# eridgd/WCT-TF

Hardware: AMD Instinct MI355X
Metric: stylized frames/sec @512x512, 5-level relu5->1 pipeline, alpha=0.8 (higher is better)
Workload: dtype f16

## Files before the change

wct_tf_amd/csrc/conv_wino.hip:

```cpp
#include "common.h"
#include "conv_tile.h"

namespace {
template <int TH, int BN, int WM, int WN>
struct WinoShape {
  static constexpr int PR = TH / 2;
  static constexpr int MT = (PR / 2) / WM;
  static constexpr int NT = (BN / 32) / WN;
  static constexpr int G = 256 / PR;
  static constexpr int SL = (72 + G - 1) / G;
  static constexpr int PATCH_BYTES = PR * 4 * PITCH * 64;
  static_assert(PR % 2 == 0 && (PR / 2) % WM == 0 && 256 % PR == 0 && WM * WN == 4, "tile shape");
  static constexpr int DUMP_OFF = 2 * PATCH_BYTES;
  static constexpr int BIAS_OFF = DUMP_OFF + 8192;
  static size_t patch_lds_bytes() { return 2 * (size_t)PATCH_BYTES; }
  static size_t lds_bytes(int cout) { return BIAS_OFF + 4 * (size_t)cout; }
};

__device__ __forceinline__ half8 pk_sub(half8 a, half8 b) {
  u32x4 ua = __builtin_bit_cast(u32x4, a), ub = __builtin_bit_cast(u32x4, b), r;
#pragma unroll
  for (int i = 0; i < 4; ++i) {
    unsigned o;
    asm("v_pk_add_f16 %0, %1, %2 neg_lo:[0,1] neg_hi:[0,1]" : "=v"(o) : "v"(ua[i]), "v"(ub[i]));
    r[i] = o;
  }
  return __builtin_bit_cast(half8, r);
}

__device__ __forceinline__ half8 wino_T(const u32x4 (&raw)[4], int f) {
  const half8 d0 = __builtin_bit_cast(half8, raw[0]), d1 = __builtin_bit_cast(half8, raw[1]);
  const half8 d2 = __builtin_bit_cast(half8, raw[2]), d3 = __builtin_bit_cast(half8, raw[3]);
  return f == 0 ? pk_sub(d0, d2) : f == 1 ? d1 + d2 : f == 2 ? pk_sub(d2, d1) : pk_sub(d1, d3);
}

__device__ __forceinline__ void wino_row_offsets(ConvArgs p, int Win, int y0, int lpr, unsigned (&row_off)[4]) {
#pragma unroll
  for (int i = 0; i < 4; ++i) {
    int iy = reflect_idx(y0 + 2 * lpr - 1 + i, p.H);
    if (p.upsample) iy >>= 1;
    row_off[i] = (unsigned)(iy * Win) * p.Cin * 2;
  }
}
__device__ __forceinline__ int wino_slot_px(int slot) { return slot < 72 ? slot >> 2 : 0; }
__device__ __forceinline__ unsigned wino_col_offset(ConvArgs p, int x0, int slot) {
  int ix = reflect_idx(x0 - 1 + wino_slot_px(slot), p.W);
  if (p.upsample) ix >>= 1;
  return (unsigned)(ix * p.Cin + (slot & 3) * 8) * 2;
}
__device__ __forceinline__ unsigned wino_slot_dst(int lpr, int slot) {
  const int px = wino_slot_px(slot), piece = slot & 3;
  return ((lpr * 4 * PITCH + px) * 4 + (piece ^ ((px >> 2) & 3))) * 16;
}

template <int MT>
__device__ __forceinline__ void wino_rd_base(int (&rd_base)[3][2], int wm, int frag_px, int frag_pr, int kgrp) {
#pragma unroll
  for (int kx = 0; kx < 3; ++kx)
#pragma unroll
    for (int ks = 0; ks < 2; ++ks) {
      const int px = frag_px + kx;
      rd_base[kx][ks] = (((wm * MT * 2 + frag_pr) * 4) * PITCH + px) * 64 + (((ks * 2 + kgrp) ^ ((px >> 2) & 3)) * 16);
    }
}
__device__ __forceinline__ half8 wino_pixel_frag(const unsigned char* patch, const int (&rd_base)[3][2], int f, int kx, int ks, int mt) {
  return *reinterpret_cast<const half8*>(patch + rd_base[kx][ks] + (mt * 8 + f) * PITCH * 64);
}
template <int MT>
__device__ __forceinline__ void wino_read_b(half8 (&dst)[2][MT], const unsigned char* patch, const int (&rd_base)[3][2], int f, int kx) {
#pragma unroll
  for (int ks = 0; ks < 2; ++ks)
#pragma unroll
    for (int mt = 0; mt < MT; ++mt) dst[ks][mt] = wino_pixel_frag(patch, rd_base, f, kx, ks, mt);
}
template <int NT>
__device__ __forceinline__ void wino_wfrag(unsigned (&wfrag)[NT], int ctile0, int wn, int c16, int lane) {
#pragma unroll
  for (int nt = 0; nt < NT; ++nt) wfrag[nt] = ((ctile0 + wn * NT + nt) * 12 * c16 * 512 + lane * 8) * 2;
}
__device__ __forceinline__ int wino_w_soff(int c16, int tap12, int chunk, unsigned wt) { return (tap12 * c16 + chunk * 2) * 1024 + wt; }
__device__ __forceinline__ half8 wino_weight_frag(__amdgpu_buffer_rsrc_t w_rsrc, unsigned wfrag, int ks, int soff) {
  return __builtin_bit_cast(half8, __builtin_amdgcn_raw_buffer_load_b128(w_rsrc, wfrag + ks * 1024, soff, 0));
}
template <int NT>
__device__ __forceinline__ void wino_load_w(half8 (&dst)[NT][2], __amdgpu_buffer_rsrc_t w_rsrc, const unsigned (&wfrag)[NT], int soff) {
#pragma unroll
  for (int nt = 0; nt < NT; ++nt)
#pragma unroll
    for (int ks = 0; ks < 2; ++ks) dst[nt][ks] = wino_weight_frag(w_rsrc, wfrag[nt], ks, soff);
}

template <int MT, int NT>
__device__ __forceinline__ void wino_init_acc(f32x16 (&acc)[4][NT][MT], const f32x4 (&bv)[NT][4]) {
#pragma unroll
  for (int nt = 0; nt < NT; ++nt)
#pragma unroll
    for (int f = 0; f < 4; ++f)
#pragma unroll
      for (int mt = 0; mt < MT; ++mt)
#pragma unroll
        for (int r = 0; r < 16; ++r) acc[f][nt][mt][r] = f == 1 ? bv[nt][r >> 2][r & 3] : 0.f;
}

template <int MT, int NT>
__device__ __forceinline__ void wino_epilogue(ConvArgs p, f32x16 (&acc)[4][NT][MT], int b, int y0, int x0, int n0, int wm, int wn,
                                              int frag_px, int frag_pr, int kgrp, int relu) {
  constexpr int OOB = (int)0x80000000u;
  const int Ho = p.pool ? (p.H + 1) / 2 : p.H, Wo = p.pool ? (p.W + 1) / 2 : p.W;
  const unsigned img_elems = (unsigned)Ho * Wo * p.Cout;
  const __amdgpu_buffer_rsrc_t r16 = __builtin_amdgcn_make_buffer_rsrc((void*)(p.y16 + (size_t)b * img_elems), 0, img_elems * 2, 0x00020000);
  const float lo1 = relu ? 0.f : -__builtin_inff();
  const h2 lo2 = {(half_t)lo1, (half_t)lo1};
  const h2 zero2 = {(half_t)0.f, (half_t)0.f};
  const int ox = x0 + frag_px;
  const int chan = n0 + wn * NT * 32;
#pragma unroll
  for (int mt = 0; mt < MT; ++mt) {
    const int oy = y0 + ((wm * MT + mt) * 2 + frag_pr) * 2;
    const bool in0 = (oy < p.H) & (ox < p.W), in1 = (oy + 1 < p.H) & (ox < p.W);
    int off[2];
    if (p.pool) {
      off[0] = in0 && (frag_px & 1) == 0 ? (((oy >> 1) * Wo + (ox >> 1)) * p.Cout + chan + 8 * kgrp) * 2 : OOB;
      off[1] = OOB;
    } else {
      off[0] = in0 ? ((oy * p.W + ox) * p.Cout + chan + 8 * kgrp) * 2 : OOB;
      off[1] = in1 ? (((oy + 1) * p.W + ox) * p.Cout + chan + 8 * kgrp) * 2 : OOB;
    }
#pragma unroll
    for (int nt = 0; nt < NT; ++nt) {
      unsigned pk[2][4][2];
#pragma unroll
      for (int rq = 0; rq < 4; ++rq) {
        f32x4 e, o;
#pragma unroll
        for (int j = 0; j < 4; ++j) {
          const int r = rq * 4 + j;
          const float m0 = acc[0][nt][mt][r], m1 = acc[1][nt][mt][r], m2 = acc[2][nt][mt][r], m3 = acc[3][nt][mt][r];
          e[j] = (m0 + m1) + m2;
          o[j] = (m1 - m2) - m3;
        }
        h2 e0 = {(half_t)e[0], (half_t)e[1]}, e1 = {(half_t)e[2], (half_t)e[3]};
        h2 o0 = {(half_t)o[0], (half_t)o[1]}, o1 = {(half_t)o[2], (half_t)o[3]};
        e0 = __builtin_elementwise_max(e0, lo2); e1 = __builtin_elementwise_max(e1, lo2);
        o0 = __builtin_elementwise_max(o0, lo2); o1 = __builtin_elementwise_max(o1, lo2);
        if (p.pool) {
          h2 q[2] = {__builtin_elementwise_max(in0 ? e0 : zero2, in1 ? o0 : zero2), __builtin_elementwise_max(in0 ? e1 : zero2, in1 ? o1 : zero2)};
#pragma unroll
          for (int d = 0; d < 2; ++d) {
            const unsigned tq = __builtin_bit_cast(unsigned, q[d]);
            const h2 nb = __builtin_bit_cast(h2, __builtin_amdgcn_update_dpp(0, (int)tq, 0xB1, 0xF, 0xF, true));
            q[d] = __builtin_elementwise_max(q[d], nb);
          }
          e0 = q[0]; e1 = q[1];
        }
        pk[0][rq][0] = __builtin_bit_cast(unsigned, e0); pk[0][rq][1] = __builtin_bit_cast(unsigned, e1);
        pk[1][rq][0] = __builtin_bit_cast(unsigned, o0); pk[1][rq][1] = __builtin_bit_cast(unsigned, o1);
      }
#pragma unroll
      for (int par = 0; par < 2; ++par) {
#pragma unroll
        for (int m = 0; m < 2; ++m) {
          auto sx = __builtin_amdgcn_permlane32_swap(pk[par][2 * m][0], pk[par][2 * m + 1][0], false, false);
          auto sy = __builtin_amdgcn_permlane32_swap(pk[par][2 * m][1], pk[par][2 * m + 1][1], false, false);
          u32x4 ov = {sx[0], sy[0], sx[1], sy[1]};
          __builtin_amdgcn_raw_buffer_store_b128(ov, r16, off[par] + (nt * 32 + 16 * m) * 2, 0, 0);
        }
      }
    }
  }
}

template <int TH, int BN, int WM, int WN>
__global__ __launch_bounds__(256, 2)
void conv3x3_wino_kernel(ConvArgs p, int tiles_x, int n_tiles) {
  using S = WinoShape<TH, BN, WM, WN>;
  constexpr int MT = S::MT, NT = S::NT, G = S::G, SL = S::SL;
  constexpr int PF_TAP = 5;
  static_assert(TH == 8, "two blocks per CU: the 8-row shapes only");

  extern __shared__ __attribute__((aligned(16))) unsigned char smem[];
  const int tid = threadIdx.x, lane = tid & 63, wave = tid >> 6;
  const int wm = wave / WN, wn = wave % WN;
  int bid = blockIdx.x;
  const int ntile = bid % n_tiles;
  bid /= n_tiles;
  const int tx = bid % tiles_x, ty = bid / tiles_x;
  const int b = blockIdx.y;
  const int y0 = ty * TH, x0 = tx * TW, n0 = ntile * BN;

  const int Hin = p.upsample ? p.H / 2 : p.H;
  const int Win = p.upsample ? p.W / 2 : p.W;
  const half_t* xb = p.x + (size_t)b * Hin * Win * p.Cin;
  const __amdgpu_buffer_rsrc_t w_rsrc = __builtin_amdgcn_make_buffer_rsrc((void*)p.w_wino, 0, 0x7FFFFFFF, 0x00020000);
  const __amdgpu_buffer_rsrc_t x_rsrc = __builtin_amdgcn_make_buffer_rsrc((void*)xb, 0, 0x7FFFFFFF, 0x00020000);

  const int lpr = tid / G, ls = tid % G;
  unsigned row_off[4], col_off[SL], dst_off[SL];
  bool slot_ok[SL];
  wino_row_offsets(p, Win, y0, lpr, row_off);
#pragma unroll
  for (int j = 0; j < SL; ++j) {
    const int slot = ls + j * G;
    slot_ok[j] = slot < 72;
    col_off[j] = wino_col_offset(p, x0, slot);
    dst_off[j] = wino_slot_dst(lpr, slot);
  }
  u32x4 raw[SL][4];
  auto load_rows = [&](int chunk) {
#pragma unroll
    for (int j = 0; j < SL; ++j)
#pragma unroll
      for (int i = 0; i < 4; ++i)
        raw[j][i] = __builtin_amdgcn_raw_buffer_load_b128(x_rsrc, row_off[i] + col_off[j], chunk * BK * 2, 0);
  };
  auto park_rows = [&](int buf) {
#pragma unroll
    for (int j = 0; j < SL; ++j) {
      const half8 t0 = wino_T(raw[j], 0), t1 = wino_T(raw[j], 1), t2 = wino_T(raw[j], 2), t3 = wino_T(raw[j], 3);
      if (slot_ok[j]) {
        unsigned char* d = smem + buf * S::PATCH_BYTES + dst_off[j];
        *reinterpret_cast<half8*>(d) = t0;
        *reinterpret_cast<half8*>(d + PITCH * 64) = t1;
        *reinterpret_cast<half8*>(d + 2 * PITCH * 64) = t2;
        *reinterpret_cast<half8*>(d + 3 * PITCH * 64) = t3;
      }
    }
  };

  const int frag_px = lane & 15, frag_pr = (lane & 31) >> 4, kgrp = lane >> 5;
  int rd_base[3][2];
  wino_rd_base<MT>(rd_base, wm, frag_px, frag_pr, kgrp);
  const int c16 = p.Cin >> 4;
  unsigned wfrag[NT];
  wino_wfrag<NT>(wfrag, n0 >> 5, wn, c16, lane);
  f32x16 acc[4][NT][MT];
  f32x4 bv[NT][4];
#pragma unroll
  for (int nt = 0; nt < NT; ++nt)
#pragma unroll
    for (int rq = 0; rq < 4; ++rq) bv[nt][rq] = *reinterpret_cast<const f32x4*>(p.bias + n0 + (wn * NT + nt) * 32 + 8 * rq + 4 * kgrp);
  wino_init_acc<MT, NT>(acc, bv);

  const int n_chunks = p.Cin / BK;
  half8 wf[3][NT][2];
  half8 bf[2][2][MT];
  auto load_w = [&](half8 (&dst)[NT][2], int tap12, int chunk) { wino_load_w<NT>(dst, w_rsrc, wfrag, wino_w_soff(c16, tap12, chunk, 0)); };
  auto read_b = [&](half8 (&dst)[2][MT], int f, int kx, int buf) { wino_read_b<MT>(dst, smem + buf * S::PATCH_BYTES, rd_base, f, kx); };

  load_rows(0);
  load_w(wf[0], 0, 0);
  load_w(wf[1], 1, 0);
  park_rows(0);
  asm volatile("s_waitcnt lgkmcnt(0)\n\ts_barrier" ::: "memory");
  read_b(bf[0], 0, 0, 0);

#pragma unroll 1
  for (int pair = 0; pair < n_chunks; pair += 2) {
#pragma unroll
    for (int t = 0; t < 24; ++t) {
      const int tt = t % 12, chunk_i = pair + t / 12, buf = t / 12;
      const int f = tt / 3;
      const bool more = chunk_i + 1 < n_chunks;
      {
        const int t2 = (tt + 2) % 12;
        const int c2 = tt + 2 >= 12 ? (more ? chunk_i + 1 : chunk_i) : chunk_i;
        load_w(wf[(t + 2) % 3], t2, c2);
      }
      if (tt == PF_TAP && more) load_rows(chunk_i + 1);
      if (tt != 11) read_b(bf[(t + 1) & 1], (tt + 1) / 3, (tt + 1) % 3, buf);
      else if (more) read_b(bf[(t + 1) & 1], 0, 0, buf ^ 1);
      __builtin_amdgcn_sched_barrier(0);
#pragma unroll
      for (int ks = 0; ks < 2; ++ks)
#pragma unroll
        for (int mt = 0; mt < MT; ++mt)
#pragma unroll
          for (int nt = 0; nt < NT; ++nt)
            acc[f][nt][mt] = __builtin_amdgcn_mfma_f32_32x32x16_f16(wf[t % 3][nt][ks], bf[t & 1][ks][mt], acc[f][nt][mt], 0, 0, 0);
      __builtin_amdgcn_sched_barrier(0);
      if (tt == 10 && more) {
        park_rows(buf ^ 1);
        asm volatile("s_waitcnt lgkmcnt(0)\n\ts_barrier" ::: "memory");
      }
    }
  }

  wino_epilogue<MT, NT>(p, acc, b, y0, x0, n0, wm, wn, frag_px, frag_pr, kgrp, p.relu);
}

template <int TH, int BN, int WM, int WN>
__global__ __launch_bounds__(256, 1)
void conv3x3_wino_walk_kernel(ConvArgs p, int tiles_x, int n_tiles, int tiles_y, int n_total) {
  using S = WinoShape<TH, BN, WM, WN>;
  constexpr int MT = S::MT, NT = S::NT, G = S::G, SL = S::SL;

  extern __shared__ __attribute__((aligned(16))) unsigned char smem[];
  const int tid = threadIdx.x, lane = tid & 63, wave = tid >> 6;
  const int wave_s = __builtin_amdgcn_readfirstlane(wave);
  auto fresh_tid = [&]() {
    int v;
    asm volatile("v_mbcnt_lo_u32_b32 %0, -1, 0\n\tv_mbcnt_hi_u32_b32 %0, -1, %0" : "=v"(v));
    return wave_s * 64 + v;
  };
  const int wm = wave / WN, wn = wave % WN;
  struct Tile { int b, y0, x0, n0; };
  auto tile_at = [&](int t) {
    Tile r;
    r.n0 = (t % n_tiles) * BN;
    t /= n_tiles;
    r.x0 = (t % tiles_x) * TW;
    t /= tiles_x;
    r.y0 = (t % tiles_y) * TH;
    r.b = t / tiles_y;
    return r;
  };
  Tile cur = tile_at(blockIdx.x);

  const int Hin = p.upsample ? p.H / 2 : p.H;
  const int Win = p.upsample ? p.W / 2 : p.W;
  const __amdgpu_buffer_rsrc_t w_rsrc = __builtin_amdgcn_make_buffer_rsrc((void*)p.w_wino, 0, 0x7FFFFFFF, 0x00020000);
  auto image_rsrc = [&](int b) { return __builtin_amdgcn_make_buffer_rsrc((void*)(p.x + (size_t)b * Hin * Win * p.Cin), 0, 0x7FFFFFFF, 0x00020000); };
  __amdgpu_buffer_rsrc_t x_rsrc = image_rsrc(cur.b);

  const int lpr = tid / G, ls = tid % G;
  unsigned row_off[4], col_off[SL], dst_off[SL];
  bool slot_ok[SL];
  auto stage_from = [&](int y0, int x0) {
    const int tid_s = fresh_tid(), lpr = tid_s / G, ls = tid_s % G;
    wino_row_offsets(p, Win, y0, lpr, row_off);
#pragma unroll
    for (int j = 0; j < SL; ++j) col_off[j] = wino_col_offset(p, x0, ls + j * G);
  };
  stage_from(cur.y0, cur.x0);
#pragma unroll
  for (int j = 0; j < SL; ++j) {
    const int slot = ls + j * G;
    slot_ok[j] = slot < 72;
    dst_off[j] = wino_slot_dst(lpr, slot);
    if (!slot_ok[j]) dst_off[j] = S::DUMP_OFF + tid * 16;
  }
  u32x4 raw[SL][4];
  auto load_rows = [&](int chunk) {
#pragma unroll
    for (int j = 0; j < SL; ++j)
#pragma unroll
      for (int i = 0; i < 4; ++i)
        raw[j][i] = __builtin_amdgcn_raw_buffer_load_b128(x_rsrc, row_off[i] + col_off[j], chunk * BK * 2, 0);
  };

  const int frag_px = lane & 15, frag_pr = (lane & 31) >> 4, kgrp = lane >> 5;
  int rd_base[3][2];
  wino_rd_base<MT>(rd_base, wm, frag_px, frag_pr, kgrp);
  const int c16 = p.Cin >> 4;
  unsigned wfrag[NT];
  wino_wfrag<NT>(wfrag, 0, wn, c16, lane);
  auto wtile_off = [&](int n0) { return (unsigned)((n0 >> 5) * 12 * c16 * 1024); };

  f32x16 acc[4][NT][MT];
  const int n_chunks = p.Cin / BK;
  half8 bf[3][2][MT];

  int tile = blockIdx.x;
  Tile nxt = cur;
  unsigned wt_cur = wtile_off(cur.n0), wt_nxt = wt_cur;
  bool has_next = false;
  constexpr int WR = 4, WA = WR - 1;
  static_assert(24 % WR == 0, "ring");
  half8 wq[WR][NT][2];
  half8 tq[4];
  {
    load_rows(0);
#pragma unroll
    for (int i = 0; i < WA; ++i) wino_load_w<NT>(wq[i], w_rsrc, wfrag, wino_w_soff(c16, i, 0, wt_cur));
#pragma unroll
    for (int j = 0; j < SL; ++j) {
      unsigned char* d = smem + dst_off[j];
      *reinterpret_cast<half8*>(d) = wino_T(raw[j], 0);
      *reinterpret_cast<half8*>(d + PITCH * 64) = wino_T(raw[j], 1);
      *reinterpret_cast<half8*>(d + 2 * PITCH * 64) = wino_T(raw[j], 2);
      *reinterpret_cast<half8*>(d + 3 * PITCH * 64) = wino_T(raw[j], 3);
    }
    for (int c = tid * 4; c < p.Cout; c += 1024) *reinterpret_cast<f32x4*>(smem + S::BIAS_OFF + c * 4) = *reinterpret_cast<const f32x4*>(p.bias + c);
    asm volatile("s_waitcnt lgkmcnt(0)\n\ts_barrier" ::: "memory");
  }
#pragma unroll 1
  for (;;) {
  {
    constexpr int NM = 2 * MT * NT;
    constexpr int NR = 2 * NT + 2 * MT;
    constexpr int LT0 = 1, PT0 = 6;
    static_assert(LT0 + SL <= PT0 && PT0 + SL <= 10, "staging schedule");
    has_next = tile + (int)gridDim.x < n_total;
    wino_read_b<MT>(bf[0], smem, rd_base, 0, 0);
    wino_read_b<MT>(bf[1], smem, rd_base, 0, 1);
    {
      const int tid_b = fresh_tid(), wn = (tid_b >> 6) % WN, kgrp = (tid_b & 63) >> 5;
      f32x4 bv[NT][4];
#pragma unroll
      for (int nt = 0; nt < NT; ++nt)
#pragma unroll
        for (int rq = 0; rq < 4; ++rq) bv[nt][rq] = *reinterpret_cast<const f32x4*>(smem + S::BIAS_OFF + (cur.n0 + (wn * NT + nt) * 32 + 8 * rq + 4 * kgrp) * 4);
      wino_init_acc<MT, NT>(acc, bv);
    }
#pragma unroll 1
    for (int pair = 0;;) {
      int stage_c = pair + 2;
      unsigned stage_wt = wt_cur;
#pragma unroll
      for (int t = 0; t < 24; ++t) {
        const int tt = t % 12, chunk_i = pair + t / 12, buf = t / 12;
        const int f = tt / 3;
        if (t == 12 && pair + 2 >= n_chunks) {
          stage_c = pair + 1;
          if (has_next) {
            nxt = tile_at(tile + (int)gridDim.x);
            stage_c = 0;
            stage_wt = wt_nxt = wtile_off(nxt.n0);
            stage_from(nxt.y0, nxt.x0);
            x_rsrc = image_rsrc(nxt.b);
          }
        }
        const int chunk_n = t < 12 ? pair + 1 : stage_c;
        const unsigned wt_n = t < 12 ? wt_cur : stage_wt;
        const int t3 = (tt + WA) % 12, c3 = tt + WA >= 12 ? chunk_n : chunk_i;
        const int t1 = (tt + 2) % 12, buf1 = tt >= 10 ? buf ^ 1 : buf;
        const int soff3 = wino_w_soff(c16, t3, c3, tt + WA >= 12 ? wt_n : wt_cur);
#pragma unroll
        for (int j = 0; j < NM; ++j) {
          const int ks = j / (MT * NT), mt = (j / NT) % MT, nt = j % NT;
          acc[f][nt][mt] = __builtin_amdgcn_mfma_f32_32x32x16_f16(wq[t % WR][nt][ks], bf[t % 3][ks][mt], acc[f][nt][mt], 0, 0, 0);
#pragma unroll
          for (int k = j * NR / NM; k < (j + 1) * NR / NM; ++k) {
            if (k < 2 * NT) {
              wq[(t + WA) % WR][k / 2][k % 2] = wino_weight_frag(w_rsrc, wfrag[k / 2], k % 2, soff3);
            } else {
              const int kk = k - 2 * NT, ks1 = kk / MT, mt1 = kk % MT;
              bf[(t + 2) % 3][ks1][mt1] = wino_pixel_frag(smem + buf1 * S::PATCH_BYTES, rd_base, t1 / 3, t1 % 3, ks1, mt1);
            }
          }
          if (tt >= LT0 && tt < LT0 + SL) {
            const int sl = tt - LT0;
            if (j < 4) raw[sl][j] = __builtin_amdgcn_raw_buffer_load_b128(x_rsrc, row_off[j] + col_off[sl], chunk_n * BK * 2, 0);
          }
          if (tt >= PT0 && tt < PT0 + SL) {
            const int sl = tt - PT0;
#pragma unroll
            for (int it = j * 8 / NM; it < (j + 1) * 8 / NM; ++it) {
              const int fq = it >> 1;
              if ((it & 1) == 0) tq[fq] = wino_T(raw[sl], fq);
              else *reinterpret_cast<half8*>(smem + (buf ^ 1) * S::PATCH_BYTES * (slot_ok[sl] ? 1 : 0) + dst_off[sl] + fq * PITCH * 64) = tq[fq];
            }
          }
          __builtin_amdgcn_sched_barrier(0);
        }
        if (tt == 9) asm volatile("s_waitcnt lgkmcnt(0)\n\ts_barrier" ::: "memory");
      }
      if ((pair += 2) >= n_chunks) break;
    }
  }
  const int tid_e = fresh_tid();
  const int lane_e = tid_e & 63, wn = (tid_e >> 6) % WN, wm = (tid_e >> 6) / WN;
  int relu = p.relu;
  asm volatile("" : "+s"(relu));
  wino_epilogue<MT, NT>(p, acc, cur.b, cur.y0, cur.x0, cur.n0, wm, wn, lane_e & 15, (lane_e & 31) >> 4, lane_e >> 5, relu);
  if (!has_next) break;
  tile += gridDim.x;
  cur = nxt;
  wt_cur = wt_nxt;
  }
}

template <int TH, int BN, int WM, int WN>
int launch_wino_cfg(const ConvArgs& a, hipStream_t s) {
  const int tiles_x = cdiv(a.W, TW), tiles_y = cdiv(a.H, TH), n_tiles = a.Cout / BN;
  const size_t lds = WinoShape<TH, BN, WM, WN>::patch_lds_bytes();
  HIP_TRY(hipFuncSetAttribute(reinterpret_cast<const void*>(&conv3x3_wino_kernel<TH, BN, WM, WN>),
                              hipFuncAttributeMaxDynamicSharedMemorySize, (int)lds));
  hipLaunchKernelGGL((conv3x3_wino_kernel<TH, BN, WM, WN>), dim3(tiles_x * tiles_y * n_tiles, a.B), dim3(256), lds, s, a, tiles_x, n_tiles);
  HIP_TRY(hipGetLastError());
  return WCT_OK;
}

template <int TH, int BN, int WM, int WN>
int launch_wino_walk(const ConvArgs& a, hipStream_t s) {
  const int tiles_x = cdiv(a.W, TW), tiles_y = cdiv(a.H, TH), n_tiles = a.Cout / BN;
  const long total = (long)tiles_x * tiles_y * n_tiles * a.B;
  const size_t lds = WinoShape<TH, BN, WM, WN>::lds_bytes(a.Cout);
  int dev = 0, cus = 0;
  HIP_TRY(hipGetDevice(&dev));
  HIP_TRY(hipDeviceGetAttribute(&cus, hipDeviceAttributeMultiprocessorCount, dev));
  ARG_CHECK(cus > 0 && total < (1L << 30) && lds <= 160 * 1024);
  HIP_TRY(hipFuncSetAttribute(reinterpret_cast<const void*>(&conv3x3_wino_walk_kernel<TH, BN, WM, WN>),
                              hipFuncAttributeMaxDynamicSharedMemorySize, (int)lds));
  hipLaunchKernelGGL((conv3x3_wino_walk_kernel<TH, BN, WM, WN>), dim3((unsigned)(total < cus ? total : cus)), dim3(256), lds, s, a, tiles_x,
                     n_tiles, tiles_y, (int)total);
  HIP_TRY(hipGetLastError());
  return WCT_OK;
}
}

bool conv3x3_wino_takes(const ConvArgs& a) {
  return a.w_wino != nullptr && a.y16 != nullptr && a.y32 == nullptr && a.usum == nullptr && a.img1 == nullptr &&
         a.Cin % 64 == 0 && a.Cout % 64 == 0 && (!a.pool || a.relu);
}

int launch_conv3x3_wino(const ConvArgs& a, hipStream_t s) {
  ARG_CHECK(conv3x3_wino_takes(a) && a.H > 1 && a.W > 1 && a.B > 0);
  ARG_CHECK(!a.upsample || (a.H % 2 == 0 && a.W % 2 == 0));
  ARG_CHECK(launch_map_fits((size_t)a.H * a.W * a.Cin, 2));
  ARG_CHECK(launch_map_fits((size_t)a.H * a.W * a.Cout, 2));
  const long px16 = (long)cdiv(a.W, TW) * cdiv(a.H, 16) * a.B;
  const long px8 = (long)cdiv(a.W, TW) * cdiv(a.H, 8) * a.B;
  if (a.Cout % 128 == 0 && px16 * (a.Cout / 128) >= 256) return launch_wino_walk<16, 128, 1, 4>(a, s);
  if (a.Cout % 128 == 0 && px8 * (a.Cout / 128) >= 256) return launch_wino_cfg<8, 128, 1, 4>(a, s);
  return launch_wino_cfg<8, 64, 2, 2>(a, s);
}
```

Before: 689.0.

## Stage Winograd input patches as vertical runs sharing overlapping row loads

Each thread now stages one pixel column across a run of three consecutive patch rows instead of several independent slots. It loads 2*RUN+2 input rows once and forms each 4-row Winograd window from overlapping slices, replacing four separate loads per slot. This cuts global input loads and address registers in the walking kernel. The cost is a different staging schedule, with two loads per step at fixed MFMA slots, and possible idle threads when the task count is below 256.

```diff
diff --git a/wct_tf_amd/csrc/conv_wino.hip b/wct_tf_amd/csrc/conv_wino.hip
--- a/wct_tf_amd/csrc/conv_wino.hip
+++ b/wct_tf_amd/csrc/conv_wino.hip
@@ -34,10 +34,11 @@
   return f == 0 ? pk_sub(d0, d2) : f == 1 ? d1 + d2 : f == 2 ? pk_sub(d2, d1) : pk_sub(d1, d3);
 }
 
-__device__ __forceinline__ void wino_row_offsets(ConvArgs p, int Win, int y0, int lpr, unsigned (&row_off)[4]) {
-#pragma unroll
-  for (int i = 0; i < 4; ++i) {
-    int iy = reflect_idx(y0 + 2 * lpr - 1 + i, p.H);
+template <int N>
+__device__ __forceinline__ void wino_row_offsets(ConvArgs p, int Win, int y0, int first, unsigned (&row_off)[N]) {
+#pragma unroll
+  for (int i = 0; i < N; ++i) {
+    int iy = reflect_idx(y0 + first - 1 + i, p.H);
     if (p.upsample) iy >>= 1;
     row_off[i] = (unsigned)(iy * Win) * p.Cin * 2;
   }
@@ -197,7 +198,7 @@
   const int lpr = tid / G, ls = tid % G;
   unsigned row_off[4], col_off[SL], dst_off[SL];
   bool slot_ok[SL];
-  wino_row_offsets(p, Win, y0, lpr, row_off);
+  wino_row_offsets(p, Win, y0, 2 * lpr, row_off);
 #pragma unroll
   for (int j = 0; j < SL; ++j) {
     const int slot = ls + j * G;
@@ -292,7 +293,7 @@
 __global__ __launch_bounds__(256, 1)
 void conv3x3_wino_walk_kernel(ConvArgs p, int tiles_x, int n_tiles, int tiles_y, int n_total) {
   using S = WinoShape<TH, BN, WM, WN>;
-  constexpr int MT = S::MT, NT = S::NT, G = S::G, SL = S::SL;
+  constexpr int MT = S::MT, NT = S::NT;
 
   extern __shared__ __attribute__((aligned(16))) unsigned char smem[];
   const int tid = threadIdx.x, lane = tid & 63, wave = tid >> 6;
@@ -322,31 +323,28 @@
   auto image_rsrc = [&](int b) { return __builtin_amdgcn_make_buffer_rsrc((void*)(p.x + (size_t)b * Hin * Win * p.Cin), 0, 0x7FFFFFFF, 0x00020000); };
   __amdgpu_buffer_rsrc_t x_rsrc = image_rsrc(cur.b);
 
-  const int lpr = tid / G, ls = tid % G;
-  unsigned row_off[4], col_off[SL], dst_off[SL];
-  bool slot_ok[SL];
+  constexpr int RUN = 3, NRAW = 2 * RUN + 2, TASKS = ((S::PR + RUN - 1) / RUN) * 72;
+  static_assert(TASKS <= 256, "one task per thread");
+  unsigned row_off[NRAW], col_off, dst_off[RUN];
+  bool park_ok[RUN];
   auto stage_from = [&](int y0, int x0) {
-    const int tid_s = fresh_tid(), lpr = tid_s / G, ls = tid_s % G;
-    wino_row_offsets(p, Win, y0, lpr, row_off);
-#pragma unroll
-    for (int j = 0; j < SL; ++j) col_off[j] = wino_col_offset(p, x0, ls + j * G);
+    const int tid_s = fresh_tid(), g = tid_s < TASKS ? tid_s / 72 : TASKS / 72 - 1, s = tid_s % 72;
+    wino_row_offsets(p, Win, y0, 2 * RUN * g, row_off);
+    col_off = wino_col_offset(p, x0, s);
   };
   stage_from(cur.y0, cur.x0);
 #pragma unroll
-  for (int j = 0; j < SL; ++j) {
-    const int slot = ls + j * G;
-    slot_ok[j] = slot < 72;
-    dst_off[j] = wino_slot_dst(lpr, slot);
-    if (!slot_ok[j]) dst_off[j] = S::DUMP_OFF + tid * 16;
-  }
-  u32x4 raw[SL][4];
+  for (int j = 0; j < RUN; ++j) {
+    const int lpr = tid / 72 * RUN + j;
+    park_ok[j] = lpr < S::PR;
+    dst_off[j] = park_ok[j] ? wino_slot_dst(lpr, tid % 72) : S::DUMP_OFF + tid * 16;
+  }
+  u32x4 raw[NRAW];
   auto load_rows = [&](int chunk) {
 #pragma unroll
-    for (int j = 0; j < SL; ++j)
-#pragma unroll
-      for (int i = 0; i < 4; ++i)
-        raw[j][i] = __builtin_amdgcn_raw_buffer_load_b128(x_rsrc, row_off[i] + col_off[j], chunk * BK * 2, 0);
+    for (int i = 0; i < NRAW; ++i) raw[i] = __builtin_amdgcn_raw_buffer_load_b128(x_rsrc, row_off[i] + col_off, chunk * BK * 2, 0);
   };
+  auto window = [&](int j) -> const u32x4 (&)[4] { return *reinterpret_cast<const u32x4 (*)[4]>(&raw[2 * j]); };
 
   const int frag_px = lane & 15, frag_pr = (lane & 31) >> 4, kgrp = lane >> 5;
   int rd_base[3][2];
@@ -373,12 +371,12 @@
 #pragma unroll
     for (int i = 0; i < WA; ++i) wino_load_w<NT>(wq[i], w_rsrc, wfrag, wino_w_soff(c16, i, 0, wt_cur));
 #pragma unroll
-    for (int j = 0; j < SL; ++j) {
+    for (int j = 0; j < RUN; ++j) {
       unsigned char* d = smem + dst_off[j];
-      *reinterpret_cast<half8*>(d) = wino_T(raw[j], 0);
-      *reinterpret_cast<half8*>(d + PITCH * 64) = wino_T(raw[j], 1);
-      *reinterpret_cast<half8*>(d + 2 * PITCH * 64) = wino_T(raw[j], 2);
-      *reinterpret_cast<half8*>(d + 3 * PITCH * 64) = wino_T(raw[j], 3);
+      *reinterpret_cast<half8*>(d) = wino_T(window(j), 0);
+      *reinterpret_cast<half8*>(d + PITCH * 64) = wino_T(window(j), 1);
+      *reinterpret_cast<half8*>(d + 2 * PITCH * 64) = wino_T(window(j), 2);
+      *reinterpret_cast<half8*>(d + 3 * PITCH * 64) = wino_T(window(j), 3);
     }
     for (int c = tid * 4; c < p.Cout; c += 1024) *reinterpret_cast<f32x4*>(smem + S::BIAS_OFF + c * 4) = *reinterpret_cast<const f32x4*>(p.bias + c);
     asm volatile("s_waitcnt lgkmcnt(0)\n\ts_barrier" ::: "memory");
@@ -388,8 +386,8 @@
   {
     constexpr int NM = 2 * MT * NT;
     constexpr int NR = 2 * NT + 2 * MT;
-    constexpr int LT0 = 1, PT0 = 6;
-    static_assert(LT0 + SL <= PT0 && PT0 + SL <= 10, "staging schedule");
+    constexpr int LT0 = 1, LJA = 2, LJB = 5, PT0 = 6;
+    static_assert(LJB < NM && LT0 + NRAW / 2 <= PT0 && PT0 + RUN <= 10, "staging schedule");
     has_next = tile + (int)gridDim.x < n_total;
     wino_read_b<MT>(bf[0], smem, rd_base, 0, 0);
     wino_read_b<MT>(bf[1], smem, rd_base, 0, 1);
@@ -438,17 +436,17 @@
               bf[(t + 2) % 3][ks1][mt1] = wino_pixel_frag(smem + buf1 * S::PATCH_BYTES, rd_base, t1 / 3, t1 % 3, ks1, mt1);
             }
           }
-          if (tt >= LT0 && tt < LT0 + SL) {
-            const int sl = tt - LT0;
-            if (j < 4) raw[sl][j] = __builtin_amdgcn_raw_buffer_load_b128(x_rsrc, row_off[j] + col_off[sl], chunk_n * BK * 2, 0);
+          if (tt >= LT0 && tt < LT0 + NRAW / 2 && (j == LJA || j == LJB)) {
+            const int i = (tt - LT0) * 2 + (j == LJB);
+            raw[i] = __builtin_amdgcn_raw_buffer_load_b128(x_rsrc, row_off[i] + col_off, chunk_n * BK * 2, 0);
           }
-          if (tt >= PT0 && tt < PT0 + SL) {
-            const int sl = tt - PT0;
+          if (tt >= PT0 && tt < PT0 + RUN) {
+            const int jr = tt - PT0;
 #pragma unroll
             for (int it = j * 8 / NM; it < (j + 1) * 8 / NM; ++it) {
               const int fq = it >> 1;
-              if ((it & 1) == 0) tq[fq] = wino_T(raw[sl], fq);
-              else *reinterpret_cast<half8*>(smem + (buf ^ 1) * S::PATCH_BYTES * (slot_ok[sl] ? 1 : 0) + dst_off[sl] + fq * PITCH * 64) = tq[fq];
+              if ((it & 1) == 0) tq[fq] = wino_T(window(jr), fq);
+              else *reinterpret_cast<half8*>(smem + (buf ^ 1) * S::PATCH_BYTES * (park_ok[jr] ? 1 : 0) + dst_off[jr] + fq * PITCH * 64) = tq[fq];
             }
           }
           __builtin_amdgcn_sched_barrier(0);
```

Result: no change. 693.1 (median of 6 runs) (+0.6%).
